# steineggerlab/unicore

Measured on AMD Instinct MI355X. Metric: 3Di alignments/sec (cluster path), higher is better.
Workload: dtype u16

## Files before the change

unicore_amd/csrc/uc_kmer_filter.hip:

```cpp
#include <hip/hip_runtime.h>

#include <algorithm>
#include <cstdlib>
#include <cstring>
#include <type_traits>

#include <rocprim/rocprim.hpp>

#include "uc_prefilter_internal.h"

namespace uc {

template <bool C>
__device__ __forceinline__ void ent_decode(const void *ent, uint32_t idx, const KeyFmt &fmt, uint32_t &t, uint32_t &pos) {
    if (C) {
        const uint32_t e = ((const uint32_t *)ent)[idx];
        t = (e >> (fmt.dbits - 1)) + fmt.tbase;
        pos = e & ((1u << (fmt.dbits - 1)) - 1u);
    } else {
        const uint64_t e = ((const uint64_t *)ent)[idx];
        t = (uint32_t)(e >> 16);
        pos = (uint32_t)(e & 0xFFFF);
    }
}

__global__ void __launch_bounds__(256) expand_kernel(const DeviceDb db, uint32_t qbegin, uint32_t qend, uint32_t p0, RunList runs,
                                                     uint64_t n_runs, const void *ent, KeyFmt fmt,
                                                     unsigned long long *key_cursor, uint64_t *keys, uint64_t key_cap) {
    __shared__ uint64_t s_pref[257];
    __shared__ uint64_t s_qb[256];
    __shared__ uint32_t s_e0[256];
    __shared__ int32_t s_i[256];
    __shared__ uint64_t s_wsum[4];
    __shared__ unsigned long long s_base;
    const int tid = threadIdx.x, lane = tid & 63, wv = tid >> 6;
    for (uint64_t tile = blockIdx.x; tile * 256 < n_runs; tile += gridDim.x) {
        const uint64_t r = tile * 256 + tid;
        uint64_t c = 0;
        if (r < n_runs) {
            const uint64_t rv = runs.val[r];
            c = rv >> 32;
            const uint32_t p = p0 + runs.pidx[r];
            const uint32_t s = find_seq(db.off, qbegin, qend, p);
            s_e0[tid] = (uint32_t)rv;
            s_i[tid] = (int32_t)(p - db.off[s]) + fmt.dbias;
            s_qb[tid] = (uint64_t)(s - qbegin) << (fmt.tbits + fmt.dbits);
        }
        uint64_t inc = c;
        for (int o = 1; o < 64; o <<= 1) {
            const uint64_t up = __shfl_up(inc, o, 64);
            if (lane >= o) inc += up;
        }
        if (lane == 63) s_wsum[wv] = inc;
        __syncthreads();
        uint64_t woff = 0;
        for (int w = 0; w < wv; w++) woff += s_wsum[w];
        s_pref[tid] = woff + inc - c;
        if (tid == 255) {
            const uint64_t total = woff + inc;
            s_pref[256] = total;
            s_base = total ? atomicAdd(key_cursor, (unsigned long long)total) : 0ull;
        }
        __syncthreads();
        const uint64_t total = s_pref[256], base = s_base;
        for (uint64_t k = tid; k < total; k += 256) {
            int lo = 0, hi = 256;
            while (hi - lo > 1) {
                const int mid = (lo + hi) >> 1;
                if (s_pref[mid] <= k) lo = mid; else hi = mid;
            }
            uint32_t et, epos;
            if (fmt.compact) ent_decode<true>(ent, s_e0[lo] + (uint32_t)(k - s_pref[lo]), fmt, et, epos);
            else ent_decode<false>(ent, s_e0[lo] + (uint32_t)(k - s_pref[lo]), fmt, et, epos);
            const uint64_t key = s_qb[lo] | ((uint64_t)et << fmt.dbits) | (uint64_t)(s_i[lo] - (int32_t)epos);
            if (base + k < key_cap) keys[base + k] = key;
        }
        __syncthreads();
    }
}

constexpr int FB_LOG2 = 19;
constexpr int FT = 1024;
constexpr int KPT = 4;
constexpr int FILTER_RPT = 2;
constexpr size_t filter_lds(int rpt) { return 2 * ((size_t)1 << FB_LOG2) / 8 + ((size_t)rpt * FT + 1) * 4 + (size_t)rpt * FT * 8 + 16 * 4 + 64; }

__global__ void __launch_bounds__(256) run_range_kernel(const DeviceDb db, uint32_t qbegin, uint32_t nq, uint32_t p0, const uint32_t *rpidx,
                                                        uint64_t n_runs, uint64_t *qr) {
    for (uint32_t i = blockIdx.x * 256 + threadIdx.x; i <= nq; i += gridDim.x * 256) {
        const uint32_t want = db.off[qbegin + i] - p0;
        uint64_t lo = 0, hi = n_runs;
        while (lo < hi) { const uint64_t m = (lo + hi) >> 1; if (rpidx[m] < want) lo = m + 1; else hi = m; }
        qr[i] = lo;
    }
}

__global__ void __launch_bounds__(256) run_order_key_kernel(uint32_t nq, const uint64_t *qr, uint32_t *key, uint32_t *idx) {
    for (uint32_t i = blockIdx.x * 256 + threadIdx.x; i < nq; i += gridDim.x * 256) {
        const uint64_t c = qr[i + 1] - qr[i];
        key[i] = 0xFFFFFFFFu - (uint32_t)min<uint64_t>(c, 0xFFFFFFFFull);
        idx[i] = i;
    }
}

template <bool C> struct TdType { using type = uint64_t; };
template <> struct TdType<true> { using type = uint32_t; };

template <bool C>
__global__ void __launch_bounds__(FT) filter_kernel(const DeviceDb db, uint32_t qbegin, uint32_t p0, const uint32_t *rpidx,
                                                    const uint64_t *rval, const uint64_t *qr, const uint32_t *order, const void *ent, KeyFmt fmt,
                                                    unsigned long long *region_cursor, void *region_v, uint64_t region_cap,
                                                    uint64_t *qbase, uint32_t *qsurv) {
    using TD = typename TdType<C>::type;
    struct __attribute__((aligned(4))) TD4 { TD v[KPT]; };
    TD *region = (TD *)region_v;
    extern __shared__ __attribute__((aligned(16))) uint32_t f_lds[];
    constexpr int BW = 1 << (FB_LOG2 - 5);
    constexpr int RPT = FILTER_RPT;
    constexpr int TR = RPT * FT;
    uint32_t *B1 = f_lds, *B2 = f_lds + BW;
    uint2 *s_run = (uint2 *)(f_lds + 2 * BW);
    uint32_t *s_pref = (uint32_t *)(s_run + TR);
    uint32_t *s_wsum = s_pref + TR + 1;
    uint64_t *s_misc = (uint64_t *)(((uintptr_t)(s_wsum + 16) + 7) & ~(uintptr_t)7);
    const int tid = threadIdx.x, lane = tid & 63, wv = tid >> 6;
    const uint32_t qi = order[blockIdx.x];
    const uint32_t q = qbegin + qi;
    const uint32_t plo = db.off[q] - p0;
    const uint64_t r0 = qr[qi], r1 = qr[qi + 1];
    TD *surv = region + region_cap;
    for (int w = tid; w < 2 * BW; w += FT) f_lds[w] = 0;
    if (r0 == r1) {
        if (tid == 0) { qbase[qi] = 0; qsurv[qi] = 0; }
        return;
    }

    uint64_t pf_rv[RPT] = {};
    uint32_t pf_pi[RPT] = {};
    auto prefetch_tile = [&](uint64_t tile) {
#pragma unroll
        for (int j = 0; j < RPT; j++) {
            const uint64_t r = tile + (uint64_t)RPT * tid + j;
            if (r < r1) { pf_rv[j] = rval[r]; pf_pi[j] = rpidx[r]; }
        }
    };
    auto load_tile = [&](uint64_t tile) {
        uint32_t c[RPT], csum = 0;
#pragma unroll
        for (int j = 0; j < RPT; j++) {
            const uint64_t r = tile + (uint64_t)RPT * tid + j;
            c[j] = r < r1 ? (uint32_t)(pf_rv[j] >> 32) : 0u;
            csum += c[j];
        }
        uint32_t inc = csum;
        for (int o = 1; o < 64; o <<= 1) {
            const uint32_t up = (uint32_t)__shfl_up((int)inc, o, 64);
            if (lane >= o) inc += up;
        }
        if (lane == 63) s_wsum[wv] = inc;
        __syncthreads();
        uint32_t woff = 0;
        for (int w = 0; w < wv; w++) woff += s_wsum[w];
        uint32_t pre = woff + inc - csum;
#pragma unroll
        for (int j = 0; j < RPT; j++) {
            s_pref[RPT * tid + j] = pre;
            s_run[RPT * tid + j] = make_uint2((uint32_t)pf_rv[j] - pre, (uint32_t)((int32_t)(pf_pi[j] - plo) + fmt.dbias));
            pre += c[j];
        }
        if (tid == FT - 1) s_pref[TR] = pre;
        __syncthreads();
    };
    auto locate = [&](uint32_t k4, uint32_t T, uint32_t (&idx)[KPT], int32_t (&si)[KPT]) -> int {
        int lo = 0;
#pragma unroll
        for (int step = TR / 2; step >= 1; step >>= 1)
            if (s_pref[lo + step] <= k4) lo += step;
        const int n = k4 >= T ? 0 : (T - k4 < (uint32_t)KPT ? (int)(T - k4) : KPT);
#pragma unroll
        for (int i = 0; i < KPT; i++) {
            if (i > 0 && i < n) lo += (s_pref[lo + 1] <= k4 + i) ? 1 : 0;
            const uint2 rr = s_run[lo];
            idx[i] = rr.x + (k4 + i);
            si[i] = (int32_t)rr.y;
        }
#pragma unroll
        for (int i = 1; i < KPT; i++) if (i >= n) { idx[i] = idx[0]; si[i] = si[0]; }
        return n;
    };
    auto gather = [&](const uint32_t (&idx)[KPT], typename std::conditional<C, uint32_t, uint64_t>::type (&e)[KPT]) {
#pragma unroll
        for (int i = 0; i < KPT; i++) {
            if (C) e[i] = ((const uint32_t *)ent)[idx[i]];
            else e[i] = ((const uint64_t *)ent)[idx[i]];
        }
    };
    auto to_td = [&](const typename std::conditional<C, uint32_t, uint64_t>::type (&e)[KPT], const int32_t (&si)[KPT], TD (&td)[KPT]) {
        const uint32_t pm = (1u << (fmt.dbits - 1)) - 1u;
#pragma unroll
        for (int i = 0; i < KPT; i++) {
            if (C) td[i] = (TD)((((uint32_t)e[i] >> (fmt.dbits - 1)) << fmt.dbits) | (uint32_t)(si[i] - (int32_t)((uint32_t)e[i] & pm)));
            else td[i] = (TD)((((uint64_t)e[i] >> 16) << fmt.dbits) | (uint64_t)(si[i] - (int32_t)((uint64_t)e[i] & 0xFFFF)));
        }
    };
    auto slot_of = [&](uint64_t td, uint32_t &h2) -> uint32_t {
        const uint32_t x = (uint32_t)td * 0x9E3779B1u ^ (uint32_t)(td >> 32) * 0x85EBCA6Bu;
        h2 = ((x ^ (x >> 15)) * 0x846CA68Bu) >> (32 - FB_LOG2);
        return (x * 0x2C1B3C6Du) >> (32 - FB_LOG2);
    };
    auto mark1 = [&](uint64_t td) {
        uint32_t g;
        const uint32_t h = slot_of(td, g), bit = 1u << (h & 31), gbit = 1u << (g & 31);
        const uint32_t old = atomicOr(&B1[h >> 5], bit);
        if (old & bit) atomicOr(&B2[h >> 5], bit);
        const uint32_t gold = atomicOr(&B1[g >> 5], gbit);
        if (gold & gbit) atomicOr(&B2[g >> 5], gbit);
    };
    auto twice1 = [&](uint64_t td) -> uint32_t {
        uint32_t g;
        const uint32_t h = slot_of(td, g);
        return ((B2[h >> 5] >> (h & 31)) & (B2[g >> 5] >> (g & 31))) & 1u;
    };

    {
        uint64_t part = 0;
        for (uint64_t r = r0 + tid; r < r1; r += FT) part += rval[r] >> 32;
        for (int o = 32; o > 0; o >>= 1) part += __shfl_down(part, o, 64);
        uint64_t *s_part = (uint64_t *)s_pref;
        if (lane == 0) s_part[wv] = part;
        __syncthreads();
        if (tid == 0) {
            uint64_t tot = 0;
            for (int w = 0; w < FT / 64; w++) tot += s_part[w];
            s_misc[2] = atomicAdd(region_cursor, (unsigned long long)((tot + KPT - 1) / KPT * KPT));
            ((uint32_t *)&s_misc[3])[0] = 0;
            ((uint32_t *)&s_misc[3])[1] = 0;
        }
        __syncthreads();
    }
    const uint64_t base = s_misc[2];
    uint32_t *cur = (uint32_t *)&s_misc[3];
    uint32_t total = 0;
    prefetch_tile(r0);
    for (uint64_t tile = r0; tile < r1; tile += TR) {
        load_tile(tile);
        prefetch_tile(tile + TR);
        const uint32_t T = s_pref[TR];
        using ET = typename std::conditional<C, uint32_t, uint64_t>::type;
        auto mark_store = [&](TD4 &td, int n, uint32_t k4) {
#pragma unroll
            for (int i = 0; i < KPT; i++) {
                if (i >= n) { td.v[i] = td.v[0]; continue; }
                mark1(td.v[i]);
            }
            const uint64_t w = base + total + k4;
            if (n && w + KPT <= region_cap) {
                if (n == KPT) *(TD4 *)(region + w) = td;
                else {
#pragma unroll
                    for (int i = 0; i < KPT; i++) if (i < n) region[w + i] = td.v[i];
                }
            }
        };
        for (uint32_t k4 = (uint32_t)KPT * tid; k4 < T; k4 += 2u * KPT * FT) {
            const uint32_t k4b = k4 + (uint32_t)KPT * FT;
            uint32_t ia[KPT], ib[KPT];
            int32_t sa[KPT], sb[KPT];
            const int na = locate(k4, T, ia, sa);
            const int nb = locate(k4b < T ? k4b : k4, T, ib, sb);
            ET ea[KPT], eb[KPT];
            gather(ia, ea);
            gather(ib, eb);
            TD4 ta, tb;
            to_td(ea, sa, ta.v);
            mark_store(ta, na, k4);
            to_td(eb, sb, tb.v);
            mark_store(tb, k4b < T ? nb : 0, k4b);
        }
        total += T;
        __syncthreads();
    }
    __threadfence_block();
    __syncthreads();
    const uint32_t n0 = (uint32_t)min<uint64_t>(total, region_cap > base ? region_cap - base : 0);
    const uint32_t n0r = n0;
    for (uint32_t k4 = (uint32_t)KPT * tid; k4 < n0r; k4 += 2u * KPT * FT) {
        TD4 td[2] = {};
        int nn[2];
#pragma unroll
        for (int g2 = 0; g2 < 2; g2++) {
            const uint32_t k = k4 + (uint32_t)g2 * KPT * FT;
            nn[g2] = k >= n0 ? 0 : (n0 - k < (uint32_t)KPT ? (int)(n0 - k) : KPT);
            if (nn[g2] == KPT) td[g2] = *(const TD4 *)(region + base + k);
            else {
#pragma unroll
                for (int i = 0; i < KPT; i++) if (i < nn[g2]) td[g2].v[i] = region[base + k + i];
            }
        }
        uint32_t keep = 0;
#pragma unroll
        for (int g2 = 0; g2 < 2; g2++)
#pragma unroll
            for (int i = 0; i < KPT; i++)
                if (i < nn[g2]) keep |= twice1(td[g2].v[i]) << (KPT * g2 + i);
        uint32_t rank[2 * KPT];
        uint32_t wave_total = 0;
#pragma unroll
        for (int j = 0; j < 2 * KPT; j++) {
            const uint64_t m = __builtin_amdgcn_ballot_w64((keep >> j) & 1u);
            rank[j] = wave_total + __builtin_amdgcn_mbcnt_hi((uint32_t)(m >> 32), __builtin_amdgcn_mbcnt_lo((uint32_t)m, 0u));
            wave_total += (uint32_t)__popcll(m);
        }
        if (wave_total) {
            uint32_t s0 = 0;
            if (lane == 0) s0 = atomicAdd(cur, wave_total);
            s0 = (uint32_t)__shfl((int)s0, 0, 64);
#pragma unroll
            for (int j = 0; j < 2 * KPT; j++)
                if ((keep >> j) & 1u) surv[base + s0 + rank[j]] = td[j / KPT].v[j % KPT];
        }
    }
    __threadfence_block();
    __syncthreads();
    const uint32_t n1 = *cur;
    for (int w = tid; w < 2 * BW; w += FT) f_lds[w] = 0;
    uint32_t *cur2 = cur + 1;
    __syncthreads();
    auto slot2_of = [&](uint64_t key, uint32_t &h2) -> uint32_t {
        const uint32_t x = (uint32_t)key * 0xC2B2AE35u ^ (uint32_t)(key >> 32) * 0x27D4EB2Fu;
        h2 = ((x ^ (x >> 13)) * 0x165667B1u) >> (32 - FB_LOG2);
        return (x * 0x9E3779B1u) >> (32 - FB_LOG2);
// ... 10 lines not shown
    const uint32_t n1r = (n1 + 63) / 64 * 64;
    for (uint32_t k = tid; k < n1r; k += FT) {
        TD key = 0;
        bool keep = false;
        if (k < n1) {
            key = surv[base + k];
            uint32_t g;
            const uint32_t h = slot2_of(key, g);
            keep = ((B2[h >> 5] >> (h & 31)) & (B2[g >> 5] >> (g & 31))) & 1u;
        }
        const uint64_t m = __builtin_amdgcn_ballot_w64(keep);
        if (m) {
            uint32_t s0 = 0;
            if (lane == 0) s0 = atomicAdd(cur2, (uint32_t)__popcll(m));
            s0 = (uint32_t)__shfl((int)s0, 0, 64);
            if (keep) region[base + s0 + (uint32_t)__popcll(m & ((1ull << lane) - 1ull))] = key;
        }
    }
    __syncthreads();
    if (tid == 0) { qbase[qi] = base; qsurv[qi] = *cur2; }
}

template <bool C>
__global__ void __launch_bounds__(256) compact_kernel(const void *region_v, const uint64_t *qbase, const uint32_t *qsurv,
                                                      const uint64_t *soff, uint32_t nq, KeyFmt fmt, uint64_t *out) {
    using TD = typename TdType<C>::type;
    const TD *region = (const TD *)region_v;
    const uint64_t dmask = (1ull << fmt.dbits) - 1;
    for (uint32_t b = blockIdx.x; b < nq; b += gridDim.x) {
        const uint64_t src = qbase[b], dst = soff[b];
        const uint32_t n = qsurv[b];
        const uint64_t qbits = (uint64_t)b << (fmt.tbits + fmt.dbits);
        for (uint32_t k = threadIdx.x; k < n; k += 256) {
            const uint64_t td = region[src + k];
            out[dst + k] = C ? (qbits | (((td >> fmt.dbits) + fmt.tbase) << fmt.dbits) | (td & dmask)) : (qbits | td);
        }
    }
}

uint64_t compact_u64(Engine &E, DevBuf<char> &tmp, uint32_t *cnt, uint64_t *pos, uint64_t n, const uint32_t *also, uint32_t *also_out) {
    auto in = rocprim::make_transform_iterator(cnt, WidenU32());
    rocprim_call(tmp, [&](void *t, size_t &b) { return rocprim::exclusive_scan(t, b, in, pos, (uint64_t)0, (size_t)n, rocprim::plus<uint64_t>(), E.stream); });
    uint64_t lp = 0; uint32_t lc = 0;
    UC_HIP(hipMemcpyAsync(&lp, pos + (n - 1), 8, hipMemcpyDeviceToHost, E.stream));
    UC_HIP(hipMemcpyAsync(&lc, cnt + (n - 1), 4, hipMemcpyDeviceToHost, E.stream));
    if (also) UC_HIP(hipMemcpyAsync(also_out, also, 4, hipMemcpyDeviceToHost, E.stream));
    UC_HIP(hipStreamSynchronize(E.stream));
    return lp + lc;
}

void expand_keys_filtered(Engine &E, PrefilterPass &PP, QueryBatch &B) {
    PrefilterScratch &S = *E.pre;
    const KeyFmt &fmt = PP.fmt;
    const uint32_t qa = B.qa, qp0 = B.qp0, nq = B.qb - B.qa;
    S.batch.d_qbase.reserve(nq); S.batch.d_qsurv.reserve(nq); S.batch.d_soff.reserve((size_t)nq + 1);
    const uint64_t region_cap = B.total_hits + (uint64_t)KPT * nq;
    S.batch.d_keys.reserve(fmt.compact ? region_cap : 2 * region_cap);
    S.batch.d_qr.reserve((size_t)nq + 1);
    hipLaunchKernelGGL(run_range_kernel, grid_for((uint64_t)nq + 1), dim3(256), 0, E.stream, E.ddb, qa, nq, qp0, S.batch.d_rpidx2.p, B.n_runs, S.batch.d_qr.p);
    S.batch.d_okey.reserve(nq); S.batch.d_okey2.reserve(nq); S.batch.d_oidx.reserve(nq); S.batch.d_order.reserve(nq);
    hipLaunchKernelGGL(run_order_key_kernel, grid_for(nq), dim3(256), 0, E.stream, nq, S.batch.d_qr.p, S.batch.d_okey.p, S.batch.d_oidx.p);
    rocprim_call(S.shared.d_temp, [&](void *t, size_t &b) { return rocprim::radix_sort_pairs(t, b, S.batch.d_okey.p, S.batch.d_okey2.p, S.batch.d_oidx.p, S.batch.d_order.p, (size_t)nq, 0u, 32u, E.stream); });
    auto launch = [&](auto kern) {
        static PerDeviceOnce once[2];
        once[fmt.compact ? 1 : 0]([&] { UC_HIP(hipFuncSetAttribute((const void *)kern, hipFuncAttributeMaxDynamicSharedMemorySize, (int)filter_lds(FILTER_RPT))); });
        hipLaunchKernelGGL(kern, dim3(nq), dim3(FT), filter_lds(FILTER_RPT), E.stream, E.ddb, qa, qp0, S.batch.d_rpidx2.p, S.batch.d_rval2.p, S.batch.d_qr.p, S.batch.d_order.p, PP.ent_p, fmt,
                           S.shared.d_counters.p + 5, (void *)S.batch.d_keys.p, region_cap, S.batch.d_qbase.p, S.batch.d_qsurv.p);
    };
    if (fmt.compact) launch(filter_kernel<true>);
    else launch(filter_kernel<false>);
    unsigned long long taken = 0;
    uint32_t last_rec = 0;
    const bool onchip = fmt.compact && PP.td_cap > 0;
    if (onchip) {
        S.cand.d_qcand.reserve(nq); S.cand.d_qmir.reserve(nq); S.cand.d_qrec.reserve(nq); S.cand.d_coff.reserve(nq);
        UC_HIP(hipMemsetAsync(S.shared.d_counters.p + 7, 0, 8, E.stream));
        launch_td_select(E, PP, qa, nq);
        auto rin = rocprim::make_transform_iterator(S.cand.d_qrec.p, WidenU32());
        rocprim_call(S.shared.d_temp, [&](void *t, size_t &b) { return rocprim::exclusive_scan(t, b, rin, S.cand.d_coff.p, (uint64_t)0, (size_t)nq, rocprim::plus<uint64_t>(), E.stream); });
        UC_HIP(hipMemcpyAsync(&B.n_rec, S.cand.d_coff.p + (nq - 1), 8, hipMemcpyDeviceToHost, E.stream));
        UC_HIP(hipMemcpyAsync(&taken, S.shared.d_counters.p + 7, 8, hipMemcpyDeviceToHost, E.stream));
    }
    const uint64_t n_sort = compact_u64(E, S.shared.d_temp, S.batch.d_qsurv.p, S.batch.d_soff.p, nq, onchip ? S.cand.d_qrec.p + (nq - 1) : nullptr, &last_rec);
    B.n_rec += last_rec;
    const uint64_t taken_keys = taken & ((1ull << 40) - 1);
    PP.td_queries += taken >> 40; PP.td_keys += taken_keys; PP.filt_queries += nq; PP.filt_keys += n_sort + taken_keys;
    E.td_onchip[0] += taken >> 40; E.td_onchip[1] += nq; E.td_onchip[2] += taken_keys; E.td_onchip[3] += n_sort + taken_keys;
    if (n_sort) {
        S.batch.d_keys2.reserve(2 * n_sort);
        hipLaunchKernelGGL(fmt.compact ? compact_kernel<true> : compact_kernel<false>, dim3(std::min<uint32_t>(nq, 65535u)), dim3(256), 0, E.stream,
                           (const void *)S.batch.d_keys.p, S.batch.d_qbase.p, S.batch.d_qsurv.p, S.batch.d_soff.p, nq, fmt, S.batch.d_keys2.p);
        rocprim_call(S.shared.d_temp, [&](void *t, size_t &b) { return rocprim::radix_sort_keys(t, b, S.batch.d_keys2.p, S.batch.d_keys2.p + n_sort, (size_t)n_sort, 0u, B.kbits, E.stream); });
    }
    B.sorted = S.batch.d_keys2.p + n_sort; B.n_sort = n_sort;
    E.stats.n_filtered_hits += n_sort + taken_keys;
}

void expand_keys_plain(Engine &E, PrefilterPass &PP, QueryBatch &B) {
    PrefilterScratch &S = *E.pre;
    S.batch.d_keys.reserve(B.total_hits); S.batch.d_keys2.reserve(B.total_hits);
    const RunList rl{S.batch.d_rpidx2.p, S.batch.d_rval2.p, PP.run_cap};
    hipLaunchKernelGGL(expand_kernel, grid_for(B.n_runs), dim3(256), 0, E.stream, E.ddb, B.qa, B.qb, B.qp0, rl, B.n_runs, PP.ent_p, PP.fmt,
                       S.shared.d_counters.p + 5, S.batch.d_keys.p, B.total_hits);
    rocprim_call(S.shared.d_temp, [&](void *t, size_t &b) { return rocprim::radix_sort_keys(t, b, S.batch.d_keys.p, S.batch.d_keys2.p, (size_t)B.total_hits, 0u, B.kbits, E.stream); });
    B.sorted = S.batch.d_keys2.p; B.n_sort = B.total_hits;
    E.stats.n_filtered_hits += B.n_sort;
}

void preload_kmer_filter_module() { hipFuncAttributes fa; (void)hipFuncGetAttributes(&fa, (const void *)run_range_kernel); }
}
```

unicore_amd/csrc/uc_kmer_match.hip:

```cpp
#include <hip/hip_runtime.h>

#include <algorithm>
#include <cstdlib>
#include <cstring>

#include <rocprim/rocprim.hpp>

#include "uc_prefilter_internal.h"

namespace uc {

constexpr uint32_t KMER_INVALID = 0xFFFFFFFFu;

__global__ void __launch_bounds__(256) kmer_extract_kernel(const DeviceDb db, uint32_t tbegin, uint32_t tend, KmerCfg cfg,
                                                           uint32_t p0, uint32_t p1, uint32_t *keys, uint64_t *vals,
                                                           uint32_t *vals32 , int pshift) {
    for (uint64_t idx = (uint64_t)blockIdx.x * 256 + threadIdx.x; idx < p1 - p0; idx += (uint64_t)gridDim.x * 256) {
        const uint32_t p = p0 + (uint32_t)idx;
        const uint32_t s = find_seq(db.off, tbegin, tend, p);
        const uint32_t j = p - db.off[s], len = db.len[s];
        uint32_t key = KMER_INVALID;
        if (j + cfg.span <= len && j <= 65535u) {
            uint32_t v = 0, mul = 1;
            bool ok = true;
// ... 331 lines not shown
    __host__ __device__ uint32_t operator()(uint8_t x) const { return (uint32_t)x; }
};

__global__ void __launch_bounds__(256) distinct_kmer_kernel(const uint8_t *flag, const uint32_t *kid, uint32_t *dk) {
    for (uint64_t v = (uint64_t)blockIdx.x * 256 + threadIdx.x; v < KSPACE; v += (uint64_t)gridDim.x * 256)
        if (flag[v]) dk[kid[v]] = (uint32_t)v;
}

__global__ void __launch_bounds__(256) rank_offsets_kernel(const uint32_t *rk, uint32_t n_runs, uint32_t nd, uint32_t *roff) {
    for (uint64_t k = (uint64_t)blockIdx.x * 256 + threadIdx.x; k <= nd; k += (uint64_t)gridDim.x * 256) {
        uint32_t lo = 0, hi = n_runs;
        while (lo < hi) {
            const uint32_t mid = lo + ((hi - lo) >> 1);
            if (rk[mid] < (uint32_t)k) lo = mid + 1; else hi = mid;
        }
        roff[k] = lo;
    }
}

__global__ void __launch_bounds__(256) rank_rec_kernel(const uint32_t *roff, const uint64_t *val, const uint32_t *nsim_k, uint32_t nd, RankRec *rec) {
    for (uint64_t k = (uint64_t)blockIdx.x * 256 + threadIdx.x; k < nd; k += (uint64_t)gridDim.x * 256) {
        uint64_t h = 0;
        const uint32_t r0 = roff[k], r1 = roff[k + 1];
        for (uint32_t r = r0; r < r1; r++) h += val[r] >> 32;
        RankRec x;
        x.roff = r0; x.nr = r1 - r0; x.nsim = nsim_k[k];
        x.hits = (uint32_t)min(h, (uint64_t)0xffffffffu);
        rec[k] = x;
    }
}

__global__ void __launch_bounds__(256) position_runs_kernel(const uint32_t *qk, uint32_t npos, const uint32_t *kid, const RankRec *rec, uint32_t *nr,
                                                            uint32_t *src, uint32_t *ph, unsigned long long *counters) {
    unsigned long long sims = 0;
    for (uint64_t idx = (uint64_t)blockIdx.x * 256 + threadIdx.x; idx < npos; idx += (uint64_t)gridDim.x * 256) {
        const uint32_t v = qk[idx];
        RankRec x = {0, 0, 0, 0};
        if (v != KMER_INVALID) x = rec[kid[v]];
        nr[idx] = x.nr; src[idx] = x.roff; ph[idx] = x.hits;
        sims += x.nsim;
    }
    block_add(sims, counters + 0);
}

__global__ void __launch_bounds__(256) query_totals_kernel(const uint32_t *off, uint32_t qbegin, uint32_t nq, uint32_t p0, const uint64_t *cumh,
                                                           const uint64_t *cumr, uint64_t *qh, uint64_t *qr) {
    for (uint64_t q = (uint64_t)blockIdx.x * 256 + threadIdx.x; q < nq; q += (uint64_t)gridDim.x * 256) {
        const uint32_t a = off[qbegin + q] - p0, b = off[qbegin + q + 1] - p0;
        qh[q] = cumh[b] - cumh[a];
        qr[q] = cumr[b] - cumr[a];
    }
}

__global__ void __launch_bounds__(256) position_expand_kernel(uint32_t b0, uint32_t b1, const uint32_t *nr, const uint32_t *src, const uint64_t *cumr,
                                                              const uint64_t *val, uint32_t *opidx, uint64_t *oval) {
    const int lane = threadIdx.x & 63;
    const uint64_t nwaves = (uint64_t)gridDim.x * 4, w0 = (uint64_t)blockIdx.x * 4 + (threadIdx.x >> 6);
    const uint64_t rbase = cumr[b0];
    for (uint64_t base = b0 + w0 * 64; base < b1; base += nwaves * 64) {
        const uint64_t idx = base + lane;
        uint32_t n = 0, s = 0, dst = 0;
        if (idx < b1) {
            n = nr[idx];
            if (n) { s = src[idx]; dst = (uint32_t)(cumr[idx] - rbase); }
        }
        uint64_t m = __builtin_amdgcn_ballot_w64(n != 0);
        while (m) {
            const int j = __builtin_ctzll(m);
            m &= m - 1;
            const uint32_t nj = (uint32_t)__shfl((int)n, j, 64), sj = (uint32_t)__shfl((int)s, j, 64), dj = (uint32_t)__shfl((int)dst, j, 64);
            for (uint32_t i = lane; i < nj; i += 64) {
                oval[dj + i] = val[sj + i];
                opidx[dj + i] = (uint32_t)(base + j - b0);
            }
        }
    }
}

KeyFmt key_format(const Engine &E, uint32_t tbegin, uint32_t tend) {
    KeyFmt fmt;
    const uint32_t m = std::min<uint32_t>(std::max<uint32_t>(E.max_len, 2), 65536u);
    fmt.dbits = 1;
    while ((1u << (fmt.dbits - 1)) < m) fmt.dbits++;
    fmt.dbias = 1 << (fmt.dbits - 1);
    fmt.tbits = 1;
    while ((1u << fmt.tbits) < E.hdb.n) fmt.tbits++;
    int rbits = 1;
    while ((1ull << rbits) < (uint64_t)std::max<uint32_t>(tend - tbegin, 1)) rbits++;
    fmt.compact = rbits + fmt.dbits <= 32 && !getenv("UC_PREFILTER_WIDE");
    fmt.tbase = tbegin;
    return fmt;
}

void build_index(Engine &E, PrefilterPass &PP) {
    PrefilterScratch &S = *E.pre;
    Timer t_index;
    E.timed_ms_begin();
    const uint32_t tp0 = E.h_poff[PP.tbegin], tp1 = E.h_poff[PP.tend];
    const uint32_t nres = tp1 - tp0;
    S.index.d_koff.reserve((size_t)KSPACE + 1);
    PP.fmt = key_format(E, PP.tbegin, PP.tend);
    const KeyFmt &fmt = PP.fmt;
    const size_t cap = std::max<uint32_t>(nres, 1);
    S.index.k_in.reserve(cap); S.index.k_out.reserve(cap);
    if (fmt.compact) { S.index.v_in32.reserve(cap); S.index.d_ent32.reserve(cap); PP.ent_p = S.index.d_ent32.p; }
    else { S.index.v_in.reserve(cap); S.index.d_ent.reserve(cap); PP.ent_p = S.index.d_ent.p; }
    if (nres) {
        hipLaunchKernelGGL(kmer_extract_kernel, grid_for(nres), dim3(256), 0, E.stream, E.ddb, PP.tbegin, PP.tend, PP.cfg, tp0, tp1, S.index.k_in.p,
                           fmt.compact ? nullptr : S.index.v_in.p, fmt.compact ? S.index.v_in32.p : nullptr, fmt.dbits - 1);
        if (fmt.compact)
            rocprim_call(S.shared.d_temp, [&](void *t, size_t &b) { return rocprim::radix_sort_pairs(t, b, S.index.k_in.p, S.index.k_out.p, S.index.v_in32.p, S.index.d_ent32.p, (size_t)nres, 0u, 32u, E.stream); });
        else
            rocprim_call(S.shared.d_temp, [&](void *t, size_t &b) { return rocprim::radix_sort_pairs(t, b, S.index.k_in.p, S.index.k_out.p, S.index.v_in.p, S.index.d_ent.p, (size_t)nres, 0u, 32u, E.stream); });
    }
    hipLaunchKernelGGL(kmer_offsets_kernel, grid_for((uint64_t)KSPACE + 1), dim3(256), 0, E.stream, S.index.k_out.p, nres, S.index.d_koff.p);
    S.index.d_kbits.reserve((KSPACE + 31) / 32);
    hipLaunchKernelGGL(kmer_bits_kernel, grid_for((KSPACE + 31) / 32), dim3(256), 0, E.stream, (const uint32_t *)S.index.d_koff.p, S.index.d_kbits.p);
    UC_HIP(hipMemcpyAsync(&PP.n_entries, S.index.d_koff.p + KSPACE, 4, hipMemcpyDeviceToHost, E.stream));
    UC_HIP(hipStreamSynchronize(E.stream));
    UC_HIP(hipGetLastError());
    PP.gpu_ms = E.timed_ms_end();
    E.stats.n_index_entries += PP.n_entries;
    E.stats.algorithmic_bytes[UC_ST_INDEX] += 6ull * PP.n_entries + 8ull * KSPACE;
    E.stats.stage_seconds[UC_ST_INDEX] += t_index.seconds();
}

dim3 sim_grid(uint64_t items) {
    return dim3((uint32_t)std::min<uint64_t>(std::max<uint64_t>(1, (items + 4 * SIM_MIN_WAVE_POS - 1) / (4 * SIM_MIN_WAVE_POS)), SIM_MAX_BLOCKS));
}

uint64_t distinct_runs(Engine &E, PrefilterPass &PP, const SuperBatch &SB, uint32_t nd, uint64_t &n_druns, uint64_t &drun_cap) {
// ... 83 lines not shown
    SB.h_qh.resize(nqa); SB.h_qr.resize(nqa);
    unsigned long long c0 = 0;
    UC_HIP(hipMemcpyAsync(SB.h_qh.data(), S.plan.d_qh.p, (size_t)nqa * 8, hipMemcpyDeviceToHost, E.stream));
    UC_HIP(hipMemcpyAsync(SB.h_qr.data(), S.plan.d_qrn.p, (size_t)nqa * 8, hipMemcpyDeviceToHost, E.stream));
    UC_HIP(hipMemcpyAsync(&c0, S.shared.d_counters.p, 8, hipMemcpyDeviceToHost, E.stream));
    UC_HIP(hipStreamSynchronize(E.stream));
    for (uint32_t i = 0; i < nqa; i++) plan_hits += SB.h_qh[i];
    SB.hit_cap = plan_hits > 16 * PP.HIT_CAP ? PP.HIT_CAP_BIG : PP.HIT_CAP;
    PP.gpu_ms += E.timed_ms_end();
    PP.t_kmer += t_p.seconds();
    if (sa == PP.qbegin) {
        if (PP.density_out) *PP.density_out = (double)plan_hits / std::max<uint32_t>(1, NP);
        if (PP.density_limit > 0 && E.p.min_diag_hits >= 2 && PP.tend - PP.tbegin > 1 && (double)plan_hits / std::max<uint32_t>(1, NP) > PP.density_limit)
            return {PlanStatus::too_dense, 0};
    }
    if (PP.count_sims) E.stats.n_sim_kmers += c0;
    return {PlanStatus::planned, 0};
}

bool choose_superbatch(Engine &E, PrefilterPass &PP, SuperBatch &SB, uint32_t qa) {
    for (;;) {
        const uint32_t left = PP.qend - qa;
        const uint32_t sb = SB.frac >= 1.0 ? PP.qend : qa + std::max<uint32_t>(1, std::min<uint32_t>(left, (uint32_t)(left * SB.frac)));
        const PlanResult r = plan_superbatch(E, PP, SB, qa, sb);
        if (r.status == PlanStatus::too_dense) {
            E.stats.n_index_entries -= PP.n_entries;
            E.stats.algorithmic_bytes[UC_ST_INDEX] -= 6ull * PP.n_entries + 8ull * KSPACE;
            E.stats.prefilter_kernel_ms += PP.gpu_ms;
            return false;
        }
        if (r.status == PlanStatus::too_many_runs) {
            SB.frac = (double)(sb - qa) / left * 0.8 * (double)PP.DRUN_MAX / (double)r.over_runs;
            continue;
        }
        if (SB.frac < 1.0) SB.frac = std::min(1.0, (double)(sb - qa) / std::max<uint32_t>(1, PP.qend - sb));
        return true;
    }
}

QueryBatch cut_batch(Engine &E, PrefilterPass &PP, const SuperBatch &SB, uint32_t qa) {
    PrefilterScratch &S = *E.pre;
    QueryBatch B;
    B.qa = B.qb = qa;
    uint64_t mirror_hits = 0;
    while (B.qb < SB.end && B.qb - qa < (1u << 23) - 1) {
        const uint64_t h = SB.h_qh[B.qb - SB.begin], r = SB.h_qr[B.qb - SB.begin];
        if (B.qb > qa && (B.total_hits + h > SB.hit_cap || B.n_runs + r > RUN_MAX)) break;
        B.total_hits += h; B.n_runs += r;
        if (B.qb >= PP.mirror_q0) mirror_hits += h;
        B.qb++;
    }
    if (B.n_runs >= (1ull << 32)) fail(UC_ERR_GENERIC, "query %u alone produces %llu index ranges", qa, (unsigned long long)B.n_runs);
    B.qp0 = E.h_poff[qa]; B.qp1 = E.h_poff[B.qb]; B.nq_res = B.qp1 - B.qp0;
    PP.run_cap = std::max<uint64_t>(PP.run_cap, B.n_runs);
    S.batch.d_rpidx2.reserve(PP.run_cap); S.batch.d_rval2.reserve(PP.run_cap);
    UC_HIP(hipMemsetAsync(S.shared.d_counters.p + 3, 0, 32, E.stream));
    if (B.n_runs)
        hipLaunchKernelGGL(position_expand_kernel, grid_for(B.nq_res), dim3(256), 0, E.stream, B.qp0 - SB.P0, B.qp1 - SB.P0, S.plan.d_nr.p, S.plan.d_src.p, S.plan.d_cumr.p, S.plan.d_drv2.p,
                           S.batch.d_rpidx2.p, S.batch.d_rval2.p);
    if (B.total_hits > (1ull << 34)) fail(UC_ERR_GENERIC, "query %u alone produces %llu k-mer hits", qa, (unsigned long long)B.total_hits);
    PP.n_hits_total += B.total_hits + mirror_hits;
    unsigned qbits = 1;
    while ((1u << qbits) < B.qb - qa) qbits++;
    B.kbits = (unsigned)(PP.fmt.dbits + PP.fmt.tbits) + qbits;
    return B;
}

void preload_kmer_match_module() { hipFuncAttributes fa; (void)hipFuncGetAttributes(&fa, (const void *)kmer_extract_kernel); }
}
```

unicore_amd/csrc/uc_prefilter_internal.h:

```cpp
#pragma once
#include <hip/hip_runtime.h>

#include "uc_engine.h"

namespace uc {

struct KmerCfg {
    int koff[K];
    int span;
    int thr;
};

__device__ __forceinline__ uint32_t find_seq(const uint32_t *off, uint32_t lo, uint32_t hi, uint32_t p) {
    while (hi - lo > 1) {
        const uint32_t mid = lo + ((hi - lo) >> 1);
        if (off[mid] <= p) lo = mid; else hi = mid;
    }
    return lo;
}

struct RunList {
    uint32_t *pidx;
    uint64_t *val;
    uint64_t cap;
};

struct RankRec { uint32_t roff, nr, hits, nsim; };

struct KeyFmt {
    int dbits, tbits;
    int dbias;
    int compact;
    uint32_t tbase;
};

struct WidenU32 {
    __host__ __device__ uint64_t operator()(uint32_t x) const { return (uint64_t)x; }
};

constexpr uint32_t TDS_CAP = 8192;


#define UC_LISTS_EVERY_BUFFER(group, count) \
    static_assert(sizeof(group) == (count) * sizeof(DevBuf<char>), #group ": a buffer was added or removed; list it in each() and correct the count")

struct SharedScratch {
    DevBuf<unsigned long long> d_counters;
    DevBuf<char> d_temp;
    template <class F> void each(F &f) { f(d_counters); f(d_temp); }
};
UC_LISTS_EVERY_BUFFER(SharedScratch, 2);
struct IndexScratch {
    DevBuf<uint32_t> d_koff, k_in, k_out, d_ent32, v_in32;
    DevBuf<uint64_t> d_ent, v_in;
    DevBuf<uint32_t> d_kbits;
    template <class F> void each(F &f) { f(d_koff); f(k_in); f(k_out); f(d_ent32); f(v_in32); f(d_ent); f(v_in); f(d_kbits); }
};
UC_LISTS_EVERY_BUFFER(IndexScratch, 8);
struct BatchScratch {
    DevBuf<uint32_t> d_okey, d_okey2, d_oidx, d_order;
    DevBuf<uint32_t> d_rpidx2, d_qsurv;
    DevBuf<uint64_t> d_keys, d_keys2, d_rval2, d_qbase, d_soff, d_qr;
    template <class F> void each(F &f) {
        f(d_okey); f(d_okey2); f(d_oidx); f(d_order); f(d_rpidx2); f(d_qsurv); f(d_keys); f(d_keys2); f(d_rval2); f(d_qbase); f(d_soff); f(d_qr);
    }
};
UC_LISTS_EVERY_BUFFER(BatchScratch, 12);
struct SelectScratch {
    DevBuf<uint32_t> d_cnt, d_flag;
    DevBuf<uint64_t> d_pos, d_skey, d_skey2;
    DevBuf<int32_t> d_cd2, d_score;
    template <class F> void each(F &f) { f(d_cnt); f(d_flag); f(d_pos); f(d_skey); f(d_skey2); f(d_cd2); f(d_score); }
};
UC_LISTS_EVERY_BUFFER(SelectScratch, 7);
struct CandScratch {
    DevBuf<uint32_t> d_cq, d_ct;
    DevBuf<int32_t> d_cd;
    DevBuf<uint8_t> d_wflag;
    DevBuf<uint32_t> d_qcand, d_qmir, d_qrec;
    DevBuf<uint64_t> d_coff;
    template <class F> void each(F &f) { f(d_cq); f(d_ct); f(d_cd); f(d_wflag); f(d_qcand); f(d_qmir); f(d_qrec); f(d_coff); }
};
UC_LISTS_EVERY_BUFFER(CandScratch, 8);
struct PlanScratch {
    DevBuf<uint8_t> d_kflag;
    DevBuf<uint32_t> d_qk, d_kid, d_dk, d_nsimk, d_drk, d_drk2, d_roff, d_nr, d_src, d_ph;
    DevBuf<uint64_t> d_drv, d_drv2, d_cumh, d_cumr, d_qh, d_qrn;
    DevBuf<RankRec> d_rec;
    template <class F> void each(F &f) {
        f(d_kflag); f(d_qk); f(d_kid); f(d_dk); f(d_nsimk); f(d_drk); f(d_drk2); f(d_roff); f(d_nr); f(d_src); f(d_ph); f(d_drv); f(d_drv2); f(d_cumh); f(d_cumr);
        f(d_qh); f(d_qrn); f(d_rec);
    }
};
UC_LISTS_EVERY_BUFFER(PlanScratch, 18);
struct MergeScratch {
    DevBuf<uint64_t> d_mkey;
    DevBuf<int32_t> d_mval;
    DevBuf<uint32_t> acc_q, acc_t, pass_q, pass_t;
    DevBuf<int32_t> acc_s, acc_d, pass_s, pass_d;
    template <class F> void each(F &f) { f(d_mkey); f(d_mval); f(acc_q); f(acc_t); f(pass_q); f(pass_t); f(acc_s); f(acc_d); f(pass_s); f(pass_d); }
};
UC_LISTS_EVERY_BUFFER(MergeScratch, 10);
UC_LISTS_EVERY_BUFFER(UngappedAllWork, 5);
#undef UC_LISTS_EVERY_BUFFER

struct PrefilterScratch {
    SharedScratch shared;
    IndexScratch index;
    BatchScratch batch;
    SelectScratch sel;
    CandScratch cand;
    PlanScratch plan;
    MergeScratch merge;
    UngappedAllWork ua;
    template <class F> void each(F f) {
        shared.each(f); index.each(f); batch.each(f); sel.each(f); cand.each(f); plan.each(f); merge.each(f);
        f(ua.score); f(ua.diag); f(ua.pairs); f(ua.prof); f(ua.prof_off);
    }
    size_t bytes() {
        size_t b = 0;
        each([&](auto &x) { b += x.cap * sizeof(*x.p); });
        return b;
    }
    void release_bytes(size_t target) {
        if (getenv("UC_TIMING")) {
            fprintf(stderr, "unicore-cluster[timing]: prefilter scratch %.1f GiB, %.1f GiB to give back before the gapped stage; buffers >= 2 GiB (index in PrefilterScratch::each: GiB):", bytes() / 1073741824.0, target / 1073741824.0);
            int i = 0;
            each([&](auto &x) { const double g = x.cap * sizeof(*x.p) / 1073741824.0; if (g >= 2.0) fprintf(stderr, " %d:%.1f", i, g); i++; });
            fprintf(stderr, "\n");
        }
        if (!target) return;
        if (target >= bytes()) { each([&](auto &x) { if (x.cap * sizeof(*x.p) >= ((size_t)1 << 30)) x.release(); }); return; }
        size_t freed = 0;
        while (freed < target) {
            size_t best = 0;
            each([&](auto &x) { best = std::max(best, x.cap * sizeof(*x.p)); });
            if (best < ((size_t)256 << 20)) break;
            bool done = false;
            each([&](auto &x) { if (!done && x.cap * sizeof(*x.p) == best) { x.release(); done = true; } });
            freed += best;
        }
    }
};

constexpr uint64_t RUN_MAX = 1ull << 29;
struct PrefilterPass {
    KmerCfg cfg;
    KeyFmt fmt;
    uint32_t tbegin = 0, tend = 0;
    uint32_t qbegin = 0, qend = 0;
    uint32_t mirror_q0 = UINT32_MAX;
    bool count_sims = false;
    double density_limit = 0.0, *density_out = nullptr;
    const void *ent_p = nullptr;
    uint32_t n_entries = 0;
    uint64_t HIT_CAP = 0, HIT_CAP_BIG = 0, DRUN_MAX = 0;
    uint64_t td_queries = 0, td_keys = 0, filt_queries = 0, filt_keys = 0;
    uint32_t td_cap = 0;
    uint64_t n_hits_total = 0, n_cand_total = 0, cand_cap = 0, run_cap = 1ull << 20;
    double t_kmer = 0, t_ung = 0, t_sel = 0, gpu_ms = 0;
};
struct SuperBatch {
    uint32_t begin = 0, end = 0;
    uint32_t P0 = 0, NP = 0;
    std::vector<uint64_t> h_qh, h_qr;
    uint64_t hit_cap = 0;
    double frac = 1.0;
};
struct QueryBatch {
    uint32_t qa = 0, qb = 0;
    uint64_t total_hits = 0, n_runs = 0;
    uint32_t qp0 = 0, qp1 = 0, nq_res = 0;
    unsigned kbits = 0;
    const uint64_t *sorted = nullptr;
    uint64_t n_sort = 0;
    uint64_t n_rec = 0;
};
enum class PlanStatus { planned, too_dense , too_many_runs  };
struct PlanResult { PlanStatus status; uint64_t over_runs; };

KeyFmt key_format(const Engine &E, uint32_t tbegin, uint32_t tend);
void build_index(Engine &E, PrefilterPass &PP);
dim3 sim_grid(uint64_t items);
uint64_t distinct_runs(Engine &E, PrefilterPass &PP, const SuperBatch &SB, uint32_t nd, uint64_t &n_druns, uint64_t &drun_cap);
PlanResult plan_superbatch(Engine &E, PrefilterPass &PP, SuperBatch &SB, uint32_t sa, uint32_t sb);
bool choose_superbatch(Engine &E, PrefilterPass &PP, SuperBatch &SB, uint32_t qa);
QueryBatch cut_batch(Engine &E, PrefilterPass &PP, const SuperBatch &SB, uint32_t qa);
uint64_t compact_u64(Engine &E, DevBuf<char> &tmp, uint32_t *cnt, uint64_t *pos, uint64_t n, const uint32_t *also = nullptr, uint32_t *also_out = nullptr);
void expand_keys_filtered(Engine &E, PrefilterPass &PP, QueryBatch &B);
void expand_keys_plain(Engine &E, PrefilterPass &PP, QueryBatch &B);
void launch_td_select(Engine &E, const PrefilterPass &PP, uint32_t qa, uint32_t nq);
uint64_t select_diagonals(Engine &E, PrefilterPass &PP, const QueryBatch &B);
void swap_hits(Engine &E, DevBuf<uint32_t> &q, DevBuf<uint32_t> &t, DevBuf<int32_t> &s, DevBuf<int32_t> &d);
void copy_hits_dev(const Engine &E, uint32_t *dq, uint32_t *dt, int32_t *ds, int32_t *dd);
void rescore_ungapped(Engine &E, PrefilterPass &PP, uint64_t n_cand);
void select_and_append(Engine &E, PrefilterPass &PP, uint64_t n_cand);

}
```

Baseline: 25.17 million.

## Read k-mer runs directly from plan arrays instead of materializing per-batch run lists

Removes position_expand_kernel and run_range_kernel. The filter and expand kernels now locate each run by binary search over the cumulative run counts (cumr) and read values straight from the distinct-run arrays. The filter kernel caches a subsampled prefix in LDS for the search, takes its region reservation from the precomputed qh instead of a reduction pass, and issues the next-tile prefetch after the first gathers. This saves a global write and reread of the run arrays and two launches, at the cost of extra search work and LDS per block.

```diff
diff --git a/unicore_amd/csrc/uc_kmer_filter.hip b/unicore_amd/csrc/uc_kmer_filter.hip
--- a/unicore_amd/csrc/uc_kmer_filter.hip
+++ b/unicore_amd/csrc/uc_kmer_filter.hip
@@ -24,9 +24,9 @@
     }
 }
 
-__global__ void __launch_bounds__(256) expand_kernel(const DeviceDb db, uint32_t qbegin, uint32_t qend, uint32_t p0, RunList runs,
-                                                     uint64_t n_runs, const void *ent, KeyFmt fmt,
-                                                     unsigned long long *key_cursor, uint64_t *keys, uint64_t key_cap) {
+__global__ void __launch_bounds__(256) expand_kernel(const DeviceDb db, uint32_t qbegin, uint32_t qend, uint32_t P0, uint32_t b0, uint32_t b1,
+                                                     const uint32_t *src, const uint64_t *cumr, const uint64_t *drv, uint64_t n_runs, const void *ent,
+                                                     KeyFmt fmt, unsigned long long *key_cursor, uint64_t *keys, uint64_t key_cap) {
     __shared__ uint64_t s_pref[257];
     __shared__ uint64_t s_qb[256];
     __shared__ uint32_t s_e0[256];
@@ -34,13 +34,19 @@
     __shared__ uint64_t s_wsum[4];
     __shared__ unsigned long long s_base;
     const int tid = threadIdx.x, lane = tid & 63, wv = tid >> 6;
+    const uint64_t rbase = cumr[b0];
     for (uint64_t tile = blockIdx.x; tile * 256 < n_runs; tile += gridDim.x) {
         const uint64_t r = tile * 256 + tid;
         uint64_t c = 0;
         if (r < n_runs) {
-            const uint64_t rv = runs.val[r];
+            uint32_t lo = b0, hi = b1;
+            while (hi - lo > 1) {
+                const uint32_t mid = lo + ((hi - lo) >> 1);
+                if (cumr[mid] - rbase <= r) lo = mid; else hi = mid;
+            }
+            const uint64_t rv = drv[src[lo] + (uint32_t)(r - (cumr[lo] - rbase))];
             c = rv >> 32;
-            const uint32_t p = p0 + runs.pidx[r];
+            const uint32_t p = P0 + lo;
             const uint32_t s = find_seq(db.off, qbegin, qend, p);
             s_e0[tid] = (uint32_t)rv;
             s_i[tid] = (int32_t)(p - db.off[s]) + fmt.dbias;
@@ -83,21 +89,15 @@
 constexpr int FT = 1024;
 constexpr int KPT = 4;
 constexpr int FILTER_RPT = 2;
-constexpr size_t filter_lds(int rpt) { return 2 * ((size_t)1 << FB_LOG2) / 8 + ((size_t)rpt * FT + 1) * 4 + (size_t)rpt * FT * 8 + 16 * 4 + 64; }
-
-__global__ void __launch_bounds__(256) run_range_kernel(const DeviceDb db, uint32_t qbegin, uint32_t nq, uint32_t p0, const uint32_t *rpidx,
-                                                        uint64_t n_runs, uint64_t *qr) {
-    for (uint32_t i = blockIdx.x * 256 + threadIdx.x; i <= nq; i += gridDim.x * 256) {
-        const uint32_t want = db.off[qbegin + i] - p0;
-        uint64_t lo = 0, hi = n_runs;
-        while (lo < hi) { const uint64_t m = (lo + hi) >> 1; if (rpidx[m] < want) lo = m + 1; else hi = m; }
-        qr[i] = lo;
-    }
-}
-
-__global__ void __launch_bounds__(256) run_order_key_kernel(uint32_t nq, const uint64_t *qr, uint32_t *key, uint32_t *idx) {
+constexpr int FILTER_PW = 1000;
+constexpr size_t filter_lds(int rpt) {
+    return 2 * ((size_t)1 << FB_LOG2) / 8 + ((size_t)rpt * FT + 1) * 4 + (size_t)rpt * FT * 8 + 16 * 4 + 64 + ((size_t)FILTER_PW + 1) * 4 + (size_t)FILTER_PW * 4;
+}
+static_assert(filter_lds(FILTER_RPT) <= 160 * 1024, "filter_kernel: one workgroup must fit the CU's LDS");
+
+__global__ void __launch_bounds__(256) run_order_key_kernel(uint32_t nq, const uint64_t *qrn, uint32_t *key, uint32_t *idx) {
     for (uint32_t i = blockIdx.x * 256 + threadIdx.x; i < nq; i += gridDim.x * 256) {
-        const uint64_t c = qr[i + 1] - qr[i];
+        const uint64_t c = qrn[i];
         key[i] = 0xFFFFFFFFu - (uint32_t)min<uint64_t>(c, 0xFFFFFFFFull);
         idx[i] = i;
     }
@@ -107,8 +107,8 @@
 template <> struct TdType<true> { using type = uint32_t; };
 
 template <bool C>
-__global__ void __launch_bounds__(FT) filter_kernel(const DeviceDb db, uint32_t qbegin, uint32_t p0, const uint32_t *rpidx,
-                                                    const uint64_t *rval, const uint64_t *qr, const uint32_t *order, const void *ent, KeyFmt fmt,
+__global__ void __launch_bounds__(FT) filter_kernel(const DeviceDb db, uint32_t qbegin, uint32_t P0, const uint32_t *psrc, const uint64_t *cumr,
+                                                    const uint64_t *drv, const uint64_t *qh, const uint32_t *order, const void *ent, KeyFmt fmt,
                                                     unsigned long long *region_cursor, void *region_v, uint64_t region_cap,
                                                     uint64_t *qbase, uint32_t *qsurv) {
     using TD = typename TdType<C>::type;
@@ -123,25 +123,54 @@
     uint32_t *s_pref = (uint32_t *)(s_run + TR);
     uint32_t *s_wsum = s_pref + TR + 1;
     uint64_t *s_misc = (uint64_t *)(((uintptr_t)(s_wsum + 16) + 7) & ~(uintptr_t)7);
+    uint32_t *s_pp = (uint32_t *)(s_misc + 4);
+    uint32_t *s_src = s_pp + FILTER_PW + 1;
     const int tid = threadIdx.x, lane = tid & 63, wv = tid >> 6;
     const uint32_t qi = order[blockIdx.x];
     const uint32_t q = qbegin + qi;
-    const uint32_t plo = db.off[q] - p0;
-    const uint64_t r0 = qr[qi], r1 = qr[qi + 1];
+    const uint32_t pq = db.off[q] - P0, L = db.off[q + 1] - db.off[q];
+    const uint64_t c0 = cumr[pq];
+    const uint64_t r0 = 0, r1 = cumr[pq + L] - c0;
     TD *surv = region + region_cap;
     for (int w = tid; w < 2 * BW; w += FT) f_lds[w] = 0;
     if (r0 == r1) {
         if (tid == 0) { qbase[qi] = 0; qsurv[qi] = 0; }
         return;
     }
+    int sh = 0;
+    while (((L + (1u << sh) - 1) >> sh) > (uint32_t)FILTER_PW) sh++;
+    const int ns = (int)((L + (1u << sh) - 1) >> sh);
+    for (int i = tid; i < ns; i += FT) {
+        s_pp[i] = (uint32_t)(cumr[pq + ((uint32_t)i << sh)] - c0);
+        if (sh == 0) s_src[i] = psrc[pq + i];
+    }
 
     uint64_t pf_rv[RPT] = {};
     uint32_t pf_pi[RPT] = {};
     auto prefetch_tile = [&](uint64_t tile) {
+        int lo = 0, hi = ns;
+        if (tile + (uint64_t)RPT * tid < r1)
+            while (hi - lo > 1) {
+                const int mid = (lo + hi) >> 1;
+                if (s_pp[mid] <= (uint32_t)(tile + (uint64_t)RPT * tid)) lo = mid; else hi = mid;
+            }
 #pragma unroll
         for (int j = 0; j < RPT; j++) {
             const uint64_t r = tile + (uint64_t)RPT * tid + j;
-            if (r < r1) { pf_rv[j] = rval[r]; pf_pi[j] = rpidx[r]; }
+            if (r < r1) {
+                if (j) while (lo + 1 < ns && s_pp[lo + 1] <= (uint32_t)r) lo++;
+                uint32_t pos = (uint32_t)lo << sh, pre = s_pp[lo], first;
+                if (sh) {
+                    uint32_t phi = min(pos + (1u << sh), L);
+                    while (phi - pos > 1) {
+                        const uint32_t mid = pos + ((phi - pos) >> 1), v = (uint32_t)(cumr[pq + mid] - c0);
+                        if (v <= (uint32_t)r) { pos = mid; pre = v; } else phi = mid;
+                    }
+                    first = psrc[pq + pos];
+                } else first = s_src[pos];
+                pf_rv[j] = drv[first + ((uint32_t)r - pre)];
+                pf_pi[j] = pos;
+            }
         }
     };
     auto load_tile = [&](uint64_t tile) {
@@ -165,7 +194,7 @@
 #pragma unroll
         for (int j = 0; j < RPT; j++) {
             s_pref[RPT * tid + j] = pre;
-            s_run[RPT * tid + j] = make_uint2((uint32_t)pf_rv[j] - pre, (uint32_t)((int32_t)(pf_pi[j] - plo) + fmt.dbias));
+            s_run[RPT * tid + j] = make_uint2((uint32_t)pf_rv[j] - pre, (uint32_t)((int32_t)pf_pi[j] + fmt.dbias));
             pre += c[j];
         }
         if (tid == FT - 1) s_pref[TR] = pre;
@@ -222,29 +251,19 @@
         return ((B2[h >> 5] >> (h & 31)) & (B2[g >> 5] >> (g & 31))) & 1u;
     };
 
-    {
-        uint64_t part = 0;
-        for (uint64_t r = r0 + tid; r < r1; r += FT) part += rval[r] >> 32;
-        for (int o = 32; o > 0; o >>= 1) part += __shfl_down(part, o, 64);
-        uint64_t *s_part = (uint64_t *)s_pref;
-        if (lane == 0) s_part[wv] = part;
-        __syncthreads();
-        if (tid == 0) {
-            uint64_t tot = 0;
-            for (int w = 0; w < FT / 64; w++) tot += s_part[w];
-            s_misc[2] = atomicAdd(region_cursor, (unsigned long long)((tot + KPT - 1) / KPT * KPT));
-            ((uint32_t *)&s_misc[3])[0] = 0;
-            ((uint32_t *)&s_misc[3])[1] = 0;
-        }
-        __syncthreads();
-    }
+    if (tid == 0) {
+        s_misc[2] = atomicAdd(region_cursor, (unsigned long long)((qh[qi] + KPT - 1) / KPT * KPT));
+        ((uint32_t *)&s_misc[3])[0] = 0;
+        ((uint32_t *)&s_misc[3])[1] = 0;
+    }
+    __syncthreads();
     const uint64_t base = s_misc[2];
     uint32_t *cur = (uint32_t *)&s_misc[3];
     uint32_t total = 0;
     prefetch_tile(r0);
     for (uint64_t tile = r0; tile < r1; tile += TR) {
         load_tile(tile);
-        prefetch_tile(tile + TR);
+        bool fetched = false;
         const uint32_t T = s_pref[TR];
         using ET = typename std::conditional<C, uint32_t, uint64_t>::type;
         auto mark_store = [&](TD4 &td, int n, uint32_t k4) {
@@ -271,12 +290,14 @@
             ET ea[KPT], eb[KPT];
             gather(ia, ea);
             gather(ib, eb);
+            if (!fetched) { prefetch_tile(tile + TR); fetched = true; }
             TD4 ta, tb;
             to_td(ea, sa, ta.v);
             mark_store(ta, na, k4);
             to_td(eb, sb, tb.v);
             mark_store(tb, k4b < T ? nb : 0, k4b);
         }
+        if (!fetched) prefetch_tile(tile + TR);
         total += T;
         __syncthreads();
     }
@@ -393,19 +414,17 @@
 void expand_keys_filtered(Engine &E, PrefilterPass &PP, QueryBatch &B) {
     PrefilterScratch &S = *E.pre;
     const KeyFmt &fmt = PP.fmt;
-    const uint32_t qa = B.qa, qp0 = B.qp0, nq = B.qb - B.qa;
+    const uint32_t qa = B.qa, nq = B.qb - B.qa;
     S.batch.d_qbase.reserve(nq); S.batch.d_qsurv.reserve(nq); S.batch.d_soff.reserve((size_t)nq + 1);
     const uint64_t region_cap = B.total_hits + (uint64_t)KPT * nq;
     S.batch.d_keys.reserve(fmt.compact ? region_cap : 2 * region_cap);
-    S.batch.d_qr.reserve((size_t)nq + 1);
-    hipLaunchKernelGGL(run_range_kernel, grid_for((uint64_t)nq + 1), dim3(256), 0, E.stream, E.ddb, qa, nq, qp0, S.batch.d_rpidx2.p, B.n_runs, S.batch.d_qr.p);
     S.batch.d_okey.reserve(nq); S.batch.d_okey2.reserve(nq); S.batch.d_oidx.reserve(nq); S.batch.d_order.reserve(nq);
-    hipLaunchKernelGGL(run_order_key_kernel, grid_for(nq), dim3(256), 0, E.stream, nq, S.batch.d_qr.p, S.batch.d_okey.p, S.batch.d_oidx.p);
+    hipLaunchKernelGGL(run_order_key_kernel, grid_for(nq), dim3(256), 0, E.stream, nq, S.plan.d_qrn.p + (qa - B.plan_q0), S.batch.d_okey.p, S.batch.d_oidx.p);
     rocprim_call(S.shared.d_temp, [&](void *t, size_t &b) { return rocprim::radix_sort_pairs(t, b, S.batch.d_okey.p, S.batch.d_okey2.p, S.batch.d_oidx.p, S.batch.d_order.p, (size_t)nq, 0u, 32u, E.stream); });
     auto launch = [&](auto kern) {
         static PerDeviceOnce once[2];
         once[fmt.compact ? 1 : 0]([&] { UC_HIP(hipFuncSetAttribute((const void *)kern, hipFuncAttributeMaxDynamicSharedMemorySize, (int)filter_lds(FILTER_RPT))); });
-        hipLaunchKernelGGL(kern, dim3(nq), dim3(FT), filter_lds(FILTER_RPT), E.stream, E.ddb, qa, qp0, S.batch.d_rpidx2.p, S.batch.d_rval2.p, S.batch.d_qr.p, S.batch.d_order.p, PP.ent_p, fmt,
+        hipLaunchKernelGGL(kern, dim3(nq), dim3(FT), filter_lds(FILTER_RPT), E.stream, E.ddb, qa, B.plan_p0, S.plan.d_src.p, S.plan.d_cumr.p, S.plan.d_drv2.p, S.plan.d_qh.p + (qa - B.plan_q0), S.batch.d_order.p, PP.ent_p, fmt,
                            S.shared.d_counters.p + 5, (void *)S.batch.d_keys.p, region_cap, S.batch.d_qbase.p, S.batch.d_qsurv.p);
     };
     if (fmt.compact) launch(filter_kernel<true>);
@@ -440,13 +459,13 @@
 void expand_keys_plain(Engine &E, PrefilterPass &PP, QueryBatch &B) {
     PrefilterScratch &S = *E.pre;
     S.batch.d_keys.reserve(B.total_hits); S.batch.d_keys2.reserve(B.total_hits);
-    const RunList rl{S.batch.d_rpidx2.p, S.batch.d_rval2.p, PP.run_cap};
-    hipLaunchKernelGGL(expand_kernel, grid_for(B.n_runs), dim3(256), 0, E.stream, E.ddb, B.qa, B.qb, B.qp0, rl, B.n_runs, PP.ent_p, PP.fmt,
+    hipLaunchKernelGGL(expand_kernel, grid_for(B.n_runs), dim3(256), 0, E.stream, E.ddb, B.qa, B.qb, B.plan_p0, B.qp0 - B.plan_p0, B.qp1 - B.plan_p0,
+                       S.plan.d_src.p, S.plan.d_cumr.p, S.plan.d_drv2.p, B.n_runs, PP.ent_p, PP.fmt,
                        S.shared.d_counters.p + 5, S.batch.d_keys.p, B.total_hits);
     rocprim_call(S.shared.d_temp, [&](void *t, size_t &b) { return rocprim::radix_sort_keys(t, b, S.batch.d_keys.p, S.batch.d_keys2.p, (size_t)B.total_hits, 0u, B.kbits, E.stream); });
     B.sorted = S.batch.d_keys2.p; B.n_sort = B.total_hits;
     E.stats.n_filtered_hits += B.n_sort;
 }
 
-void preload_kmer_filter_module() { hipFuncAttributes fa; (void)hipFuncGetAttributes(&fa, (const void *)run_range_kernel); }
-}
+void preload_kmer_filter_module() { hipFuncAttributes fa; (void)hipFuncGetAttributes(&fa, (const void *)run_order_key_kernel); }
+}
diff --git a/unicore_amd/csrc/uc_kmer_match.hip b/unicore_amd/csrc/uc_kmer_match.hip
--- a/unicore_amd/csrc/uc_kmer_match.hip
+++ b/unicore_amd/csrc/uc_kmer_match.hip
@@ -407,31 +407,6 @@
     }
 }
 
-__global__ void __launch_bounds__(256) position_expand_kernel(uint32_t b0, uint32_t b1, const uint32_t *nr, const uint32_t *src, const uint64_t *cumr,
-                                                              const uint64_t *val, uint32_t *opidx, uint64_t *oval) {
-    const int lane = threadIdx.x & 63;
-    const uint64_t nwaves = (uint64_t)gridDim.x * 4, w0 = (uint64_t)blockIdx.x * 4 + (threadIdx.x >> 6);
-    const uint64_t rbase = cumr[b0];
-    for (uint64_t base = b0 + w0 * 64; base < b1; base += nwaves * 64) {
-        const uint64_t idx = base + lane;
-        uint32_t n = 0, s = 0, dst = 0;
-        if (idx < b1) {
-            n = nr[idx];
-            if (n) { s = src[idx]; dst = (uint32_t)(cumr[idx] - rbase); }
-        }
-        uint64_t m = __builtin_amdgcn_ballot_w64(n != 0);
-        while (m) {
-            const int j = __builtin_ctzll(m);
-            m &= m - 1;
-            const uint32_t nj = (uint32_t)__shfl((int)n, j, 64), sj = (uint32_t)__shfl((int)s, j, 64), dj = (uint32_t)__shfl((int)dst, j, 64);
-            for (uint32_t i = lane; i < nj; i += 64) {
-                oval[dj + i] = val[sj + i];
-                opidx[dj + i] = (uint32_t)(base + j - b0);
-            }
-        }
-    }
-}
-
 KeyFmt key_format(const Engine &E, uint32_t tbegin, uint32_t tend) {
     KeyFmt fmt;
     const uint32_t m = std::min<uint32_t>(std::max<uint32_t>(E.max_len, 2), 65536u);
@@ -621,12 +596,8 @@
     }
     if (B.n_runs >= (1ull << 32)) fail(UC_ERR_GENERIC, "query %u alone produces %llu index ranges", qa, (unsigned long long)B.n_runs);
     B.qp0 = E.h_poff[qa]; B.qp1 = E.h_poff[B.qb]; B.nq_res = B.qp1 - B.qp0;
-    PP.run_cap = std::max<uint64_t>(PP.run_cap, B.n_runs);
-    S.batch.d_rpidx2.reserve(PP.run_cap); S.batch.d_rval2.reserve(PP.run_cap);
+    B.plan_p0 = SB.P0; B.plan_q0 = SB.begin;
     UC_HIP(hipMemsetAsync(S.shared.d_counters.p + 3, 0, 32, E.stream));
-    if (B.n_runs)
-        hipLaunchKernelGGL(position_expand_kernel, grid_for(B.nq_res), dim3(256), 0, E.stream, B.qp0 - SB.P0, B.qp1 - SB.P0, S.plan.d_nr.p, S.plan.d_src.p, S.plan.d_cumr.p, S.plan.d_drv2.p,
-                           S.batch.d_rpidx2.p, S.batch.d_rval2.p);
     if (B.total_hits > (1ull << 34)) fail(UC_ERR_GENERIC, "query %u alone produces %llu k-mer hits", qa, (unsigned long long)B.total_hits);
     PP.n_hits_total += B.total_hits + mirror_hits;
     unsigned qbits = 1;
diff --git a/unicore_amd/csrc/uc_prefilter_internal.h b/unicore_amd/csrc/uc_prefilter_internal.h
--- a/unicore_amd/csrc/uc_prefilter_internal.h
+++ b/unicore_amd/csrc/uc_prefilter_internal.h
@@ -59,13 +59,11 @@
 UC_LISTS_EVERY_BUFFER(IndexScratch, 8);
 struct BatchScratch {
     DevBuf<uint32_t> d_okey, d_okey2, d_oidx, d_order;
-    DevBuf<uint32_t> d_rpidx2, d_qsurv;
-    DevBuf<uint64_t> d_keys, d_keys2, d_rval2, d_qbase, d_soff, d_qr;
-    template <class F> void each(F &f) {
-        f(d_okey); f(d_okey2); f(d_oidx); f(d_order); f(d_rpidx2); f(d_qsurv); f(d_keys); f(d_keys2); f(d_rval2); f(d_qbase); f(d_soff); f(d_qr);
-    }
+    DevBuf<uint32_t> d_qsurv;
+    DevBuf<uint64_t> d_keys, d_keys2, d_qbase, d_soff;
+    template <class F> void each(F &f) { f(d_okey); f(d_okey2); f(d_oidx); f(d_order); f(d_qsurv); f(d_keys); f(d_keys2); f(d_qbase); f(d_soff); }
 };
-UC_LISTS_EVERY_BUFFER(BatchScratch, 12);
+UC_LISTS_EVERY_BUFFER(BatchScratch, 9);
 struct SelectScratch {
     DevBuf<uint32_t> d_cnt, d_flag;
     DevBuf<uint64_t> d_pos, d_skey, d_skey2;
@@ -157,7 +155,7 @@
     uint64_t HIT_CAP = 0, HIT_CAP_BIG = 0, DRUN_MAX = 0;
     uint64_t td_queries = 0, td_keys = 0, filt_queries = 0, filt_keys = 0;
     uint32_t td_cap = 0;
-    uint64_t n_hits_total = 0, n_cand_total = 0, cand_cap = 0, run_cap = 1ull << 20;
+    uint64_t n_hits_total = 0, n_cand_total = 0, cand_cap = 0;
     double t_kmer = 0, t_ung = 0, t_sel = 0, gpu_ms = 0;
 };
 struct SuperBatch {
@@ -171,6 +169,7 @@
     uint32_t qa = 0, qb = 0;
     uint64_t total_hits = 0, n_runs = 0;
     uint32_t qp0 = 0, qp1 = 0, nq_res = 0;
+    uint32_t plan_p0 = 0, plan_q0 = 0;
     unsigned kbits = 0;
     const uint64_t *sorted = nullptr;
     uint64_t n_sort = 0;
```

Measured after the change: 25.47 million, median of 6. 1.01x the previous value.
